# loicland/superpoint_graph

Measured on NVIDIA H100. Metric: spg_train_step_edges_plus_points_per_sec, higher is better.
Workload: dtype f32

## Files before the change

superpoint_graph_b200/csrc/tc_common.cuh:

```cuda
#pragma once
#include <cuda_runtime.h>
#include <stdint.h>

namespace spg {

__device__ __forceinline__ uint32_t smem_u32(const void* p) {
    return (uint32_t)__cvta_generic_to_shared(p);
}

__device__ __forceinline__ uint32_t to_tf32(float v) {
    return (__float_as_uint(v) + 0x1000u) & 0xffffe000u;
}

__device__ __forceinline__ void mbar_init(uint32_t bar, uint32_t count) {
    asm volatile("mbarrier.init.shared::cta.b64 [%0], %1;" ::"r"(bar), "r"(count));
}

__device__ __forceinline__ void mbar_wait(uint32_t bar, uint32_t parity) {
    asm volatile(
        "{\n\t"
        ".reg .pred P1;\n\t"
        "WAIT_LOOP:\n\t"
        "mbarrier.try_wait.parity.shared::cta.b64 P1, [%0], %1;\n\t"
        "@P1 bra WAIT_DONE;\n\t"
        "bra WAIT_LOOP;\n\t"
        "WAIT_DONE:\n\t"
        "}" ::"r"(bar), "r"(parity)
        : "memory");
}

__device__ __forceinline__ void mbar_arrive(uint32_t bar) {
    asm volatile("mbarrier.arrive.shared::cta.b64 _, [%0];" ::"r"(bar) : "memory");
}

__device__ __forceinline__ void mbar_expect_tx(uint32_t bar, uint32_t bytes) {
    asm volatile("mbarrier.arrive.expect_tx.shared::cta.b64 _, [%0], %1;" ::"r"(bar), "r"(bytes) : "memory");
}

__device__ __forceinline__ uint64_t wg_desc_k_sw128(uint32_t saddr) {
    return (uint64_t)((saddr >> 4) & 0x3FFFu) | ((uint64_t)1 << 16) | ((uint64_t)64 << 32) | ((uint64_t)1 << 62);
}

__device__ __forceinline__ uint32_t sw128_off(int row, int c16) {
    return (uint32_t)((row >> 3) * 1024 + (row & 7) * 128 + ((c16 ^ (row & 7)) << 4));
}

__device__ __forceinline__ void wg_fence() { asm volatile("wgmma.fence.sync.aligned;" ::: "memory"); }
__device__ __forceinline__ void wg_commit() { asm volatile("wgmma.commit_group.sync.aligned;" ::: "memory"); }
template <int N>
__device__ __forceinline__ void wg_wait() {
    asm volatile("wgmma.wait_group.sync.aligned %0;" ::"n"(N) : "memory");
}

template <int R>
__device__ __forceinline__ void wg_reg_fence(float (&d)[R]) {
#pragma unroll
    for (int i = 0; i < R; ++i) asm volatile("" : "+f"(d[i])::"memory");
}

template <int N>
__device__ __forceinline__ void wgmma_tf32(float (&d)[N / 2], uint64_t da, uint64_t db, uint32_t acc);
template <int N>
__device__ __forceinline__ void wgmma_bf16(float (&d)[N / 2], uint64_t da, uint64_t db, uint32_t acc);

template <>
__device__ __forceinline__ void wgmma_tf32<16>(float (&d)[8], uint64_t da, uint64_t db, uint32_t acc) {
    asm volatile(
        "{\n\t.reg .pred p;\n\tsetp.ne.b32 p, %10, 0;\n\t"
        "wgmma.mma_async.sync.aligned.m64n16k8.f32.tf32.tf32 {%0, %1, %2, %3, %4, %5, %6, %7}, %8, %9, p, 1, 1;\n\t}"
        : "+f"(d[0]), "+f"(d[1]), "+f"(d[2]), "+f"(d[3]), "+f"(d[4]), "+f"(d[5]), "+f"(d[6]), "+f"(d[7])
        : "l"(da), "l"(db), "r"(acc));
}

template <>
__device__ __forceinline__ void wgmma_tf32<32>(float (&d)[16], uint64_t da, uint64_t db, uint32_t acc) {
    asm volatile(
        "{\n\t.reg .pred p;\n\tsetp.ne.b32 p, %18, 0;\n\t"
        "wgmma.mma_async.sync.aligned.m64n32k8.f32.tf32.tf32 {%0, %1, %2, %3, %4, %5, %6, %7, %8, %9, %10, %11, %12, %13, %14, %15}, %16, %17, p, 1, 1;\n\t}"
        : "+f"(d[0]), "+f"(d[1]), "+f"(d[2]), "+f"(d[3]), "+f"(d[4]), "+f"(d[5]), "+f"(d[6]), "+f"(d[7]), "+f"(d[8]), "+f"(d[9]), "+f"(d[10]), "+f"(d[11]), "+f"(d[12]), "+f"(d[13]), "+f"(d[14]), "+f"(d[15])
        : "l"(da), "l"(db), "r"(acc));
}

template <>
__device__ __forceinline__ void wgmma_tf32<64>(float (&d)[32], uint64_t da, uint64_t db, uint32_t acc) {
    asm volatile(
        "{\n\t.reg .pred p;\n\tsetp.ne.b32 p, %34, 0;\n\t"
        "wgmma.mma_async.sync.aligned.m64n64k8.f32.tf32.tf32 {%0, %1, %2, %3, %4, %5, %6, %7, %8, %9, %10, %11, %12, %13, %14, %15, %16, %17, %18, %19, %20, %21, %22, %23, %24, %25, %26, %27, %28, %29, %30, %31}, %32, %33, p, 1, 1;\n\t}"
        : "+f"(d[0]), "+f"(d[1]), "+f"(d[2]), "+f"(d[3]), "+f"(d[4]), "+f"(d[5]), "+f"(d[6]), "+f"(d[7]), "+f"(d[8]), "+f"(d[9]), "+f"(d[10]), "+f"(d[11]), "+f"(d[12]), "+f"(d[13]), "+f"(d[14]), "+f"(d[15]), "+f"(d[16]), "+f"(d[17]), "+f"(d[18]), "+f"(d[19]), "+f"(d[20]), "+f"(d[21]), "+f"(d[22]), "+f"(d[23]), "+f"(d[24]), "+f"(d[25]), "+f"(d[26]), "+f"(d[27]), "+f"(d[28]), "+f"(d[29]), "+f"(d[30]), "+f"(d[31])
        : "l"(da), "l"(db), "r"(acc));
}

template <>
__device__ __forceinline__ void wgmma_tf32<128>(float (&d)[64], uint64_t da, uint64_t db, uint32_t acc) {
    asm volatile(
        "{\n\t.reg .pred p;\n\tsetp.ne.b32 p, %66, 0;\n\t"
        "wgmma.mma_async.sync.aligned.m64n128k8.f32.tf32.tf32 {%0, %1, %2, %3, %4, %5, %6, %7, %8, %9, %10, %11, %12, %13, %14, %15, %16, %17, %18, %19, %20, %21, %22, %23, %24, %25, %26, %27, %28, %29, %30, %31, %32, %33, %34, %35, %36, %37, %38, %39, %40, %41, %42, %43, %44, %45, %46, %47, %48, %49, %50, %51, %52, %53, %54, %55, %56, %57, %58, %59, %60, %61, %62, %63}, %64, %65, p, 1, 1;\n\t}"
        : "+f"(d[0]), "+f"(d[1]), "+f"(d[2]), "+f"(d[3]), "+f"(d[4]), "+f"(d[5]), "+f"(d[6]), "+f"(d[7]), "+f"(d[8]), "+f"(d[9]), "+f"(d[10]), "+f"(d[11]), "+f"(d[12]), "+f"(d[13]), "+f"(d[14]), "+f"(d[15]), "+f"(d[16]), "+f"(d[17]), "+f"(d[18]), "+f"(d[19]), "+f"(d[20]), "+f"(d[21]), "+f"(d[22]), "+f"(d[23]), "+f"(d[24]), "+f"(d[25]), "+f"(d[26]), "+f"(d[27]), "+f"(d[28]), "+f"(d[29]), "+f"(d[30]), "+f"(d[31]), "+f"(d[32]), "+f"(d[33]), "+f"(d[34]), "+f"(d[35]), "+f"(d[36]), "+f"(d[37]), "+f"(d[38]), "+f"(d[39]), "+f"(d[40]), "+f"(d[41]), "+f"(d[42]), "+f"(d[43]), "+f"(d[44]), "+f"(d[45]), "+f"(d[46]), "+f"(d[47]), "+f"(d[48]), "+f"(d[49]), "+f"(d[50]), "+f"(d[51]), "+f"(d[52]), "+f"(d[53]), "+f"(d[54]), "+f"(d[55]), "+f"(d[56]), "+f"(d[57]), "+f"(d[58]), "+f"(d[59]), "+f"(d[60]), "+f"(d[61]), "+f"(d[62]), "+f"(d[63])
        : "l"(da), "l"(db), "r"(acc));
}

template <>
__device__ __forceinline__ void wgmma_bf16<32>(float (&d)[16], uint64_t da, uint64_t db, uint32_t acc) {
    asm volatile(
        "{\n\t.reg .pred p;\n\tsetp.ne.b32 p, %18, 0;\n\t"
        "wgmma.mma_async.sync.aligned.m64n32k16.f32.bf16.bf16 {%0, %1, %2, %3, %4, %5, %6, %7, %8, %9, %10, %11, %12, %13, %14, %15}, %16, %17, p, 1, 1, 0, 0;\n\t}"
        : "+f"(d[0]), "+f"(d[1]), "+f"(d[2]), "+f"(d[3]), "+f"(d[4]), "+f"(d[5]), "+f"(d[6]), "+f"(d[7]), "+f"(d[8]), "+f"(d[9]), "+f"(d[10]), "+f"(d[11]), "+f"(d[12]), "+f"(d[13]), "+f"(d[14]), "+f"(d[15])
        : "l"(da), "l"(db), "r"(acc));
}

template <>
__device__ __forceinline__ void wgmma_bf16<64>(float (&d)[32], uint64_t da, uint64_t db, uint32_t acc) {
    asm volatile(
        "{\n\t.reg .pred p;\n\tsetp.ne.b32 p, %34, 0;\n\t"
        "wgmma.mma_async.sync.aligned.m64n64k16.f32.bf16.bf16 {%0, %1, %2, %3, %4, %5, %6, %7, %8, %9, %10, %11, %12, %13, %14, %15, %16, %17, %18, %19, %20, %21, %22, %23, %24, %25, %26, %27, %28, %29, %30, %31}, %32, %33, p, 1, 1, 0, 0;\n\t}"
        : "+f"(d[0]), "+f"(d[1]), "+f"(d[2]), "+f"(d[3]), "+f"(d[4]), "+f"(d[5]), "+f"(d[6]), "+f"(d[7]), "+f"(d[8]), "+f"(d[9]), "+f"(d[10]), "+f"(d[11]), "+f"(d[12]), "+f"(d[13]), "+f"(d[14]), "+f"(d[15]), "+f"(d[16]), "+f"(d[17]), "+f"(d[18]), "+f"(d[19]), "+f"(d[20]), "+f"(d[21]), "+f"(d[22]), "+f"(d[23]), "+f"(d[24]), "+f"(d[25]), "+f"(d[26]), "+f"(d[27]), "+f"(d[28]), "+f"(d[29]), "+f"(d[30]), "+f"(d[31])
        : "l"(da), "l"(db), "r"(acc));
}

template <>
__device__ __forceinline__ void wgmma_bf16<128>(float (&d)[64], uint64_t da, uint64_t db, uint32_t acc) {
    asm volatile(
        "{\n\t.reg .pred p;\n\tsetp.ne.b32 p, %66, 0;\n\t"
        "wgmma.mma_async.sync.aligned.m64n128k16.f32.bf16.bf16 {%0, %1, %2, %3, %4, %5, %6, %7, %8, %9, %10, %11, %12, %13, %14, %15, %16, %17, %18, %19, %20, %21, %22, %23, %24, %25, %26, %27, %28, %29, %30, %31, %32, %33, %34, %35, %36, %37, %38, %39, %40, %41, %42, %43, %44, %45, %46, %47, %48, %49, %50, %51, %52, %53, %54, %55, %56, %57, %58, %59, %60, %61, %62, %63}, %64, %65, p, 1, 1, 0, 0;\n\t}"
        : "+f"(d[0]), "+f"(d[1]), "+f"(d[2]), "+f"(d[3]), "+f"(d[4]), "+f"(d[5]), "+f"(d[6]), "+f"(d[7]), "+f"(d[8]), "+f"(d[9]), "+f"(d[10]), "+f"(d[11]), "+f"(d[12]), "+f"(d[13]), "+f"(d[14]), "+f"(d[15]), "+f"(d[16]), "+f"(d[17]), "+f"(d[18]), "+f"(d[19]), "+f"(d[20]), "+f"(d[21]), "+f"(d[22]), "+f"(d[23]), "+f"(d[24]), "+f"(d[25]), "+f"(d[26]), "+f"(d[27]), "+f"(d[28]), "+f"(d[29]), "+f"(d[30]), "+f"(d[31]), "+f"(d[32]), "+f"(d[33]), "+f"(d[34]), "+f"(d[35]), "+f"(d[36]), "+f"(d[37]), "+f"(d[38]), "+f"(d[39]), "+f"(d[40]), "+f"(d[41]), "+f"(d[42]), "+f"(d[43]), "+f"(d[44]), "+f"(d[45]), "+f"(d[46]), "+f"(d[47]), "+f"(d[48]), "+f"(d[49]), "+f"(d[50]), "+f"(d[51]), "+f"(d[52]), "+f"(d[53]), "+f"(d[54]), "+f"(d[55]), "+f"(d[56]), "+f"(d[57]), "+f"(d[58]), "+f"(d[59]), "+f"(d[60]), "+f"(d[61]), "+f"(d[62]), "+f"(d[63])
        : "l"(da), "l"(db), "r"(acc));
}


}
```

superpoint_graph_b200/csrc/tc_dw.cu:

```cuda
#include "common.cuh"
#include "tc_common.cuh"

namespace spg {

constexpr int DW_CONS_WARPS = 8, DW_PROD_WARPS = 4;
constexpr int DW_PROD_THREADS = DW_PROD_WARPS * 32;
constexpr int DW_THREADS = (DW_CONS_WARPS + DW_PROD_WARPS) * 32;
constexpr int DW_PTS = 32;
constexpr int DW_MAX_STAGES = 4;
constexpr int DW_SMEM_LIMIT = 232448;
constexpr int DW_STATIC_SMEM = 2048;

template <int CO, int CI>
struct DwCfg {
    static constexpr int A_BYTES = CO * DW_PTS * 4;
    static constexpr int B_BYTES = CI * DW_PTS * 4;
    static constexpr int STAGE_BYTES = 2 * A_BYTES + 2 * B_BYTES;
    static constexpr int FIT = (DW_SMEM_LIMIT - 1024 - DW_STATIC_SMEM) / STAGE_BYTES;
    static constexpr int STAGES = FIT < DW_MAX_STAGES ? FIT : DW_MAX_STAGES;
    static constexpr int SMEM = STAGES * STAGE_BYTES + 1024;
    static constexpr int A_F4 = CO * DW_PTS / 4 / DW_PROD_THREADS;
    static constexpr int B_F4 = CI * DW_PTS / 4 / DW_PROD_THREADS;
    static constexpr int PF_FIT = 24 / (A_F4 + B_F4);
    static constexpr int PF = PF_FIT < 1 ? 1 : (PF_FIT > 4 ? 4 : PF_FIT);
    static_assert(STAGES >= 2, "ring");
};

struct DwArgs {
    const float* dY;
    int64_t lddy;
    const float* P;
    int64_t ldp;
    const float *p_scale, *p_shift;
    int p_relu;
    float* partial;
    int64_t M;
    int64_t pts_per_cta;
};

template <int CO, int CI>
__global__ void __launch_bounds__(DW_THREADS, 1) tc_dw_kernel(const DwArgs p) {
    using Cfg = DwCfg<CO, CI>;
    constexpr int WM = CO >= 128 ? CO / 2 : 64;
    constexpr int WN = CO >= 128 ? CI : CI / 2;
    constexpr int MSUB = WM / 64;
    constexpr int A_BYTES = Cfg::A_BYTES, B_BYTES = Cfg::B_BYTES, STAGE_BYTES = Cfg::STAGE_BYTES;
    constexpr int STAGES = Cfg::STAGES, PF = Cfg::PF, A_F4 = Cfg::A_F4, B_F4 = Cfg::B_F4;
    static_assert(CO % 64 == 0 && CI % 32 == 0 && CI <= 128 && CO <= 256, "shape");

    extern __shared__ __align__(1024) uint8_t smem_raw[];
    uint8_t* smem = reinterpret_cast<uint8_t*>((reinterpret_cast<uintptr_t>(smem_raw) + 1023) & ~(uintptr_t)1023);
    __shared__ __align__(8) uint64_t bars[2 * DW_MAX_STAGES];
    __shared__ __align__(16) float sc_s[128], sh_s[128];
    static_assert(sizeof(bars) + sizeof(sc_s) + sizeof(sh_s) <= DW_STATIC_SMEM, "static shared memory");

    const int t = threadIdx.x;
    const int warp = t >> 5, lane = t & 31;
    const uint32_t bars_u32 = smem_u32(&bars[0]);
    auto bar_full = [&](int s) { return bars_u32 + 8u * (uint32_t)s; };
    auto bar_empty = [&](int s) { return bars_u32 + 8u * (uint32_t)(DW_MAX_STAGES + s); };
    if (t == 0) {
#pragma unroll
        for (int s = 0; s < STAGES; ++s) {
            mbar_init(bar_full(s), DW_PROD_WARPS);
            mbar_init(bar_empty(s), DW_CONS_WARPS);
        }
        asm volatile("fence.mbarrier_init.release.cluster;" ::: "memory");
    }
    SPG_PDL_ENTRY();

    const int64_t m_beg = (int64_t)blockIdx.x * p.pts_per_cta;
    const int64_t m_end = min(p.M, m_beg + p.pts_per_cta);
    const int nchunks = m_beg < m_end ? (int)((m_end - m_beg + DW_PTS - 1) / DW_PTS) : 0;

    const int ptid = t - DW_CONS_WARPS * 32;
    const int pt = (ptid >> 5) * 8 + (lane & 7), c40 = lane >> 3;
    float4 q[PF][A_F4 + B_F4];
    auto load_chunk = [&](int ch, float4 (&dst)[A_F4 + B_F4]) {
        const int64_t row = m_beg + (int64_t)ch * DW_PTS + pt;
        const bool ok = row < m_end;
        const float4* ga = reinterpret_cast<const float4*>(p.dY + row * p.lddy) + c40;
        const float4* gb = reinterpret_cast<const float4*>(p.P + row * p.ldp) + c40;
#pragma unroll
        for (int j = 0; j < A_F4; ++j) dst[j] = ok ? __ldg(ga + 4 * j) : make_float4(0.f, 0.f, 0.f, 0.f);
#pragma unroll
        for (int j = 0; j < B_F4; ++j) dst[A_F4 + j] = ok ? __ldg(gb + 4 * j) : make_float4(0.f, 0.f, 0.f, 0.f);
    };
    if (ptid >= 0) {
#pragma unroll
        for (int d = 0; d < PF; ++d) load_chunk(d, q[d]);
    }
    if (t < CI) {
        sc_s[t] = p.p_scale ? p.p_scale[t] : 1.f;
        sh_s[t] = p.p_shift ? p.p_shift[t] : 0.f;
    }
    __syncthreads();

    if (warp >= DW_CONS_WARPS) {
        const bool pro = p.p_scale || p.p_shift || p.p_relu;
        uint32_t soff[4];
#pragma unroll
        for (int e = 0; e < 4; ++e) soff[e] = sw128_off(4 * c40 + e, pt >> 2) + (uint32_t)(pt & 3) * 4u;
        auto st_shared = [](uint32_t addr, uint32_t v) {
            asm volatile("st.shared.b32 [%0], %1;" ::"r"(addr), "r"(v) : "memory");
        };
        auto split_store = [&](const uint32_t (&base)[4], uint32_t hi_off, uint32_t lo, int j, float4 v) {
            const float vv[4] = {v.x, v.y, v.z, v.w};
#pragma unroll
            for (int e = 0; e < 4; ++e) {
                const uint32_t addr = base[e] + hi_off + 2048u * (uint32_t)j;
                const uint32_t hi = to_tf32(vv[e]);
                st_shared(addr, hi);
                st_shared(addr + lo, to_tf32(vv[e] - __uint_as_float(hi)));
            }
        };
        const uint32_t smem_u = smem_u32(smem);
        int ch = 0, s = 0;
        uint32_t use = 0;
        auto produce = [&](float4 (&cur)[A_F4 + B_F4]) {
            if (use > 0) mbar_wait(bar_empty(s), (use - 1) & 1);
            uint32_t base[4];
#pragma unroll
            for (int e = 0; e < 4; ++e) base[e] = smem_u + (uint32_t)s * STAGE_BYTES + soff[e];
            const bool affine = pro && m_beg + (int64_t)ch * DW_PTS + pt < m_end;
#pragma unroll
            for (int j = 0; j < A_F4; ++j) split_store(base, 0u, A_BYTES, j, cur[j]);
#pragma unroll
            for (int j = 0; j < B_F4; ++j) {
                float4 v = cur[A_F4 + j];
                if (affine) {
                    const float4 sc = *reinterpret_cast<const float4*>(sc_s + (c40 + 4 * j) * 4);
                    const float4 sh = *reinterpret_cast<const float4*>(sh_s + (c40 + 4 * j) * 4);
                    v.x = fmaf(v.x, sc.x, sh.x);
                    v.y = fmaf(v.y, sc.y, sh.y);
                    v.z = fmaf(v.z, sc.z, sh.z);
                    v.w = fmaf(v.w, sc.w, sh.w);
                    if (p.p_relu) {
                        v.x = fmaxf(v.x, 0.f);
                        v.y = fmaxf(v.y, 0.f);
                        v.z = fmaxf(v.z, 0.f);
                        v.w = fmaxf(v.w, 0.f);
                    }
                }
                split_store(base, 2 * A_BYTES, B_BYTES, j, v);
            }
            load_chunk(ch + PF, cur);
            asm volatile("fence.proxy.async.shared::cta;" ::: "memory");
            __syncwarp();
            if (lane == 0) mbar_arrive(bar_full(s));
            ++ch;
            if (++s == STAGES) {
                s = 0;
                ++use;
            }
        };
        while (ch < nchunks) {
#pragma unroll
            for (int u = 0; u < PF; ++u) {
                produce(q[u]);
                if (ch >= nchunks) break;
            }
        }
    } else {
        const int g = warp >> 2, wl = warp & 3;
        float acc[MSUB][WN / 2];
#pragma unroll
        for (int m = 0; m < MSUB; ++m)
#pragma unroll
            for (int i = 0; i < WN / 2; ++i) acc[m][i] = 0.f;
        const int row_g = CO >= 128 ? g * WM : 0;
        const int col_g = CO >= 128 ? 0 : g * WN;
        const uint32_t smem_u = smem_u32(smem);

        int s = 0, s_prev = 0;
        uint32_t phase = 0;
        for (int ch = 0; ch < nchunks; ++ch) {
            mbar_wait(bar_full(s), phase);
            const uint32_t a_hi = smem_u + (uint32_t)s * STAGE_BYTES;
            const uint32_t ah = a_hi + (uint32_t)row_g * 128u, al = ah + A_BYTES;
            const uint32_t bh = a_hi + 2 * A_BYTES + (uint32_t)col_g * 128u, bl = bh + B_BYTES;
#pragma unroll
            for (int m = 0; m < MSUB; ++m) wg_reg_fence(acc[m]);
            wg_fence();
#pragma unroll
            for (int kb = 0; kb < DW_PTS / 8; ++kb) {
                const uint64_t dbh = wg_desc_k_sw128(bh + kb * 32), dbl = wg_desc_k_sw128(bl + kb * 32);
#pragma unroll
                for (int m = 0; m < MSUB; ++m) {
                    const uint64_t dah = wg_desc_k_sw128(ah + m * 64 * 128 + kb * 32);
                    const uint64_t dal = wg_desc_k_sw128(al + m * 64 * 128 + kb * 32);
                    wgmma_tf32<WN>(acc[m], dah, dbh, 1u);
                    wgmma_tf32<WN>(acc[m], dal, dbh, 1u);
                    wgmma_tf32<WN>(acc[m], dah, dbl, 1u);
                }
            }
            wg_commit();
            if (ch > 0) {
                wg_wait<1>();
                __syncwarp();
                if (lane == 0) mbar_arrive(bar_empty(s_prev));
            }
            s_prev = s;
            if (++s == STAGES) {
                s = 0;
                phase ^= 1u;
            }
        }
        wg_wait<0>();
#pragma unroll
        for (int m = 0; m < MSUB; ++m) wg_reg_fence(acc[m]);

        float* out = p.partial + (int64_t)blockIdx.x * CO * CI;
        const int r = lane >> 2, cq = 2 * (lane & 3);
#pragma unroll
        for (int m = 0; m < MSUB; ++m) {
            const int row = row_g + m * 64 + wl * 16 + r;
#pragma unroll
            for (int j = 0; j < WN / 8; ++j) {
                const int col = col_g + 8 * j + cq;
                *reinterpret_cast<float2*>(out + (int64_t)row * CI + col) =
                    make_float2(acc[m][4 * j], acc[m][4 * j + 1]);
                *reinterpret_cast<float2*>(out + (int64_t)(row + 8) * CI + col) =
                    make_float2(acc[m][4 * j + 2], acc[m][4 * j + 3]);
            }
        }
    }
}

template <int CO, int CI>
static int launch_dw(const DwArgs& a, int ctas, cudaStream_t s) {
    constexpr int smem = DwCfg<CO, CI>::SMEM;
    cudaError_t e = cudaFuncSetAttribute(tc_dw_kernel<CO, CI>, cudaFuncAttributeMaxDynamicSharedMemorySize, smem);
    if (e != cudaSuccess) return (int)e;
    SPG_LAUNCH(K_TC_DW, s, (tc_dw_kernel<CO, CI>), (unsigned)ctas, DW_THREADS, smem, a);
    return launch_status();
}

}

using namespace spg;

extern "C" {

int spg_tc_dw_supported(int64_t M, int co, int ci) {
    const bool co_ok = (co == 64 || co == 128 || co == 256);
    const bool ci_ok = (ci == 32 || ci == 64 || ci == 128);
    return (M >= DW_PTS && co_ok && ci_ok) ? 1 : 0;
}

int spg_tc_dw_ctas(int64_t M) {
    int64_t chunks = ceil_div64(M, DW_PTS);
    int64_t ctas = chunks < kNumSMs ? chunks : kNumSMs;
    return (int)(ctas < 1 ? 1 : ctas);
}

int spg_tc_dw(const float* dY, int64_t lddy, const float* P, int64_t ldp, const float* p_scale,
              const float* p_shift, int p_relu, float* dW, float* workspace, int64_t M, int co, int ci,
              spg_stream_t stream) {
    if (!dY || !P || !dW || !workspace || M <= 0) return SPG_E_BADARG;
    if (!spg_tc_dw_supported(M, co, ci)) return SPG_E_UNSUPPORTED;
    if ((lddy & 3) || (ldp & 3) || lddy < co || ldp < ci) return SPG_E_ALIGN;
    if (((uintptr_t)dY | (uintptr_t)P | (uintptr_t)workspace | (uintptr_t)p_scale | (uintptr_t)p_shift) & 15)
        return SPG_E_ALIGN;
    const int ctas = spg_tc_dw_ctas(M);
    DwArgs a;
    a.dY = dY; a.lddy = lddy; a.P = P; a.ldp = ldp; a.p_scale = p_scale; a.p_shift = p_shift;
    a.p_relu = p_relu; a.partial = workspace; a.M = M;
    cudaStream_t s = (cudaStream_t)stream;
    a.pts_per_cta = ceil_div64(ceil_div64(M, ctas), DW_PTS) * DW_PTS;
    int rc;
#define SPG_DW_CASE(CO_, CI_) \
    if (co == CO_ && ci == CI_) rc = launch_dw<CO_, CI_>(a, ctas, s); else
    SPG_DW_CASE(64, 32) SPG_DW_CASE(64, 64) SPG_DW_CASE(64, 128) SPG_DW_CASE(128, 32)
    SPG_DW_CASE(128, 64) SPG_DW_CASE(128, 128) SPG_DW_CASE(256, 32) SPG_DW_CASE(256, 64)
    SPG_DW_CASE(256, 128) rc = SPG_E_UNSUPPORTED;
#undef SPG_DW_CASE
    if (rc) return rc;
    return spg_splitk_reduce(workspace, ctas, co, ci, nullptr, dW, ci, stream);
}

}
```

Before: 47.68 million.

## Load dY operand directly into registers for wgmma A fragments in dW kernel

The weight-gradient kernel now has consumer warps load dY straight from global memory into register A-fragments, split them into tf32 hi/lo in registers, and feed register-sourced wgmma. This drops dY staging through shared memory, so stages hold only P and the ring is a fixed 4 stages. The output row mapping is permuted to match the fragment layout, and setmaxnreg rebalances registers between producer and consumer warps for large tiles. In exchange, consumers now sit on global-load latency and carry more register pressure, and the finer per-k-step wgmma commit/wait pattern adds synchronisation.

```diff
diff --git a/superpoint_graph_b200/csrc/tc_common.cuh b/superpoint_graph_b200/csrc/tc_common.cuh
--- a/superpoint_graph_b200/csrc/tc_common.cuh
+++ b/superpoint_graph_b200/csrc/tc_common.cuh
@@ -57,6 +57,11 @@
 #pragma unroll
     for (int i = 0; i < R; ++i) asm volatile("" : "+f"(d[i])::"memory");
 }
+template <int R>
+__device__ __forceinline__ void wg_reg_fence(uint32_t (&d)[R]) {
+#pragma unroll
+    for (int i = 0; i < R; ++i) asm volatile("" : "+r"(d[i])::"memory");
+}
 
 template <int N>
 __device__ __forceinline__ void wgmma_tf32(float (&d)[N / 2], uint64_t da, uint64_t db, uint32_t acc);
@@ -99,6 +104,45 @@
         : "l"(da), "l"(db), "r"(acc));
 }
 
+template <int N>
+__device__ __forceinline__ void wgmma_tf32(float (&d)[N / 2], const uint32_t (&a)[4], uint64_t db, uint32_t acc);
+
+template <>
+__device__ __forceinline__ void wgmma_tf32<16>(float (&d)[8], const uint32_t (&a)[4], uint64_t db, uint32_t acc) {
+    asm volatile(
+        "{\n\t.reg .pred p;\n\tsetp.ne.b32 p, %13, 0;\n\t"
+        "wgmma.mma_async.sync.aligned.m64n16k8.f32.tf32.tf32 {%0, %1, %2, %3, %4, %5, %6, %7}, {%8, %9, %10, %11}, %12, p, 1, 1;\n\t}"
+        : "+f"(d[0]), "+f"(d[1]), "+f"(d[2]), "+f"(d[3]), "+f"(d[4]), "+f"(d[5]), "+f"(d[6]), "+f"(d[7])
+        : "r"(a[0]), "r"(a[1]), "r"(a[2]), "r"(a[3]), "l"(db), "r"(acc));
+}
+
+template <>
+__device__ __forceinline__ void wgmma_tf32<32>(float (&d)[16], const uint32_t (&a)[4], uint64_t db, uint32_t acc) {
+    asm volatile(
+        "{\n\t.reg .pred p;\n\tsetp.ne.b32 p, %21, 0;\n\t"
+        "wgmma.mma_async.sync.aligned.m64n32k8.f32.tf32.tf32 {%0, %1, %2, %3, %4, %5, %6, %7, %8, %9, %10, %11, %12, %13, %14, %15}, {%16, %17, %18, %19}, %20, p, 1, 1;\n\t}"
+        : "+f"(d[0]), "+f"(d[1]), "+f"(d[2]), "+f"(d[3]), "+f"(d[4]), "+f"(d[5]), "+f"(d[6]), "+f"(d[7]), "+f"(d[8]), "+f"(d[9]), "+f"(d[10]), "+f"(d[11]), "+f"(d[12]), "+f"(d[13]), "+f"(d[14]), "+f"(d[15])
+        : "r"(a[0]), "r"(a[1]), "r"(a[2]), "r"(a[3]), "l"(db), "r"(acc));
+}
+
+template <>
+__device__ __forceinline__ void wgmma_tf32<64>(float (&d)[32], const uint32_t (&a)[4], uint64_t db, uint32_t acc) {
+    asm volatile(
+        "{\n\t.reg .pred p;\n\tsetp.ne.b32 p, %37, 0;\n\t"
+        "wgmma.mma_async.sync.aligned.m64n64k8.f32.tf32.tf32 {%0, %1, %2, %3, %4, %5, %6, %7, %8, %9, %10, %11, %12, %13, %14, %15, %16, %17, %18, %19, %20, %21, %22, %23, %24, %25, %26, %27, %28, %29, %30, %31}, {%32, %33, %34, %35}, %36, p, 1, 1;\n\t}"
+        : "+f"(d[0]), "+f"(d[1]), "+f"(d[2]), "+f"(d[3]), "+f"(d[4]), "+f"(d[5]), "+f"(d[6]), "+f"(d[7]), "+f"(d[8]), "+f"(d[9]), "+f"(d[10]), "+f"(d[11]), "+f"(d[12]), "+f"(d[13]), "+f"(d[14]), "+f"(d[15]), "+f"(d[16]), "+f"(d[17]), "+f"(d[18]), "+f"(d[19]), "+f"(d[20]), "+f"(d[21]), "+f"(d[22]), "+f"(d[23]), "+f"(d[24]), "+f"(d[25]), "+f"(d[26]), "+f"(d[27]), "+f"(d[28]), "+f"(d[29]), "+f"(d[30]), "+f"(d[31])
+        : "r"(a[0]), "r"(a[1]), "r"(a[2]), "r"(a[3]), "l"(db), "r"(acc));
+}
+
+template <>
+__device__ __forceinline__ void wgmma_tf32<128>(float (&d)[64], const uint32_t (&a)[4], uint64_t db, uint32_t acc) {
+    asm volatile(
+        "{\n\t.reg .pred p;\n\tsetp.ne.b32 p, %69, 0;\n\t"
+        "wgmma.mma_async.sync.aligned.m64n128k8.f32.tf32.tf32 {%0, %1, %2, %3, %4, %5, %6, %7, %8, %9, %10, %11, %12, %13, %14, %15, %16, %17, %18, %19, %20, %21, %22, %23, %24, %25, %26, %27, %28, %29, %30, %31, %32, %33, %34, %35, %36, %37, %38, %39, %40, %41, %42, %43, %44, %45, %46, %47, %48, %49, %50, %51, %52, %53, %54, %55, %56, %57, %58, %59, %60, %61, %62, %63}, {%64, %65, %66, %67}, %68, p, 1, 1;\n\t}"
+        : "+f"(d[0]), "+f"(d[1]), "+f"(d[2]), "+f"(d[3]), "+f"(d[4]), "+f"(d[5]), "+f"(d[6]), "+f"(d[7]), "+f"(d[8]), "+f"(d[9]), "+f"(d[10]), "+f"(d[11]), "+f"(d[12]), "+f"(d[13]), "+f"(d[14]), "+f"(d[15]), "+f"(d[16]), "+f"(d[17]), "+f"(d[18]), "+f"(d[19]), "+f"(d[20]), "+f"(d[21]), "+f"(d[22]), "+f"(d[23]), "+f"(d[24]), "+f"(d[25]), "+f"(d[26]), "+f"(d[27]), "+f"(d[28]), "+f"(d[29]), "+f"(d[30]), "+f"(d[31]), "+f"(d[32]), "+f"(d[33]), "+f"(d[34]), "+f"(d[35]), "+f"(d[36]), "+f"(d[37]), "+f"(d[38]), "+f"(d[39]), "+f"(d[40]), "+f"(d[41]), "+f"(d[42]), "+f"(d[43]), "+f"(d[44]), "+f"(d[45]), "+f"(d[46]), "+f"(d[47]), "+f"(d[48]), "+f"(d[49]), "+f"(d[50]), "+f"(d[51]), "+f"(d[52]), "+f"(d[53]), "+f"(d[54]), "+f"(d[55]), "+f"(d[56]), "+f"(d[57]), "+f"(d[58]), "+f"(d[59]), "+f"(d[60]), "+f"(d[61]), "+f"(d[62]), "+f"(d[63])
+        : "r"(a[0]), "r"(a[1]), "r"(a[2]), "r"(a[3]), "l"(db), "r"(acc));
+}
+
 template <>
 __device__ __forceinline__ void wgmma_bf16<32>(float (&d)[16], uint64_t da, uint64_t db, uint32_t acc) {
     asm volatile(
diff --git a/superpoint_graph_b200/csrc/tc_dw.cu b/superpoint_graph_b200/csrc/tc_dw.cu
--- a/superpoint_graph_b200/csrc/tc_dw.cu
+++ b/superpoint_graph_b200/csrc/tc_dw.cu
@@ -1,5 +1,7 @@
 #include "common.cuh"
 #include "tc_common.cuh"
+
+#include <type_traits>
 
 namespace spg {
 
@@ -7,23 +9,28 @@
 constexpr int DW_PROD_THREADS = DW_PROD_WARPS * 32;
 constexpr int DW_THREADS = (DW_CONS_WARPS + DW_PROD_WARPS) * 32;
 constexpr int DW_PTS = 32;
-constexpr int DW_MAX_STAGES = 4;
+constexpr int DW_KSTEPS = DW_PTS / 8;
+constexpr int DW_STAGES = 4;
 constexpr int DW_SMEM_LIMIT = 232448;
 constexpr int DW_STATIC_SMEM = 2048;
 
 template <int CO, int CI>
 struct DwCfg {
-    static constexpr int A_BYTES = CO * DW_PTS * 4;
+    static constexpr int WM = CO >= 128 ? CO / 2 : 64;
+    static constexpr int WN = CO >= 128 ? CI : CI / 2;
+    static constexpr int MSUB = WM / 64;
     static constexpr int B_BYTES = CI * DW_PTS * 4;
-    static constexpr int STAGE_BYTES = 2 * A_BYTES + 2 * B_BYTES;
-    static constexpr int FIT = (DW_SMEM_LIMIT - 1024 - DW_STATIC_SMEM) / STAGE_BYTES;
-    static constexpr int STAGES = FIT < DW_MAX_STAGES ? FIT : DW_MAX_STAGES;
-    static constexpr int SMEM = STAGES * STAGE_BYTES + 1024;
-    static constexpr int A_F4 = CO * DW_PTS / 4 / DW_PROD_THREADS;
+    static constexpr int STAGE_BYTES = 2 * B_BYTES;
+    static constexpr int SMEM = DW_STAGES * STAGE_BYTES + 1024;
+    static_assert(SMEM + DW_STATIC_SMEM <= DW_SMEM_LIMIT, "ring");
     static constexpr int B_F4 = CI * DW_PTS / 4 / DW_PROD_THREADS;
-    static constexpr int PF_FIT = 24 / (A_F4 + B_F4);
+    static constexpr bool REG_SPLIT = WM * WN > 128 * 64;
+    static constexpr int CONS_REGS = 224, PROD_REGS = 56;
+    static constexpr int PF_FIT = REG_SPLIT ? 1 : 24 / B_F4;
     static constexpr int PF = PF_FIT < 1 ? 1 : (PF_FIT > 4 ? 4 : PF_FIT);
-    static_assert(STAGES >= 2, "ring");
+    static constexpr int HL = WN * MSUB <= 64 ? 4 : 2;
+    static constexpr int RAW = MSUB == 1 ? 2 * DW_KSTEPS : 2;
+    static_assert(DW_KSTEPS % HL == 0 && (DW_KSTEPS % RAW == 0 || RAW == 2 * DW_KSTEPS), "A fragment rings");
 };
 
 struct DwArgs {
@@ -41,16 +48,14 @@
 template <int CO, int CI>
 __global__ void __launch_bounds__(DW_THREADS, 1) tc_dw_kernel(const DwArgs p) {
     using Cfg = DwCfg<CO, CI>;
-    constexpr int WM = CO >= 128 ? CO / 2 : 64;
-    constexpr int WN = CO >= 128 ? CI : CI / 2;
-    constexpr int MSUB = WM / 64;
-    constexpr int A_BYTES = Cfg::A_BYTES, B_BYTES = Cfg::B_BYTES, STAGE_BYTES = Cfg::STAGE_BYTES;
-    constexpr int STAGES = Cfg::STAGES, PF = Cfg::PF, A_F4 = Cfg::A_F4, B_F4 = Cfg::B_F4;
+    constexpr int WM = Cfg::WM, WN = Cfg::WN, MSUB = Cfg::MSUB;
+    constexpr int B_BYTES = Cfg::B_BYTES, STAGE_BYTES = Cfg::STAGE_BYTES;
+    constexpr int PF = Cfg::PF, B_F4 = Cfg::B_F4, HL = Cfg::HL, RAW = Cfg::RAW;
     static_assert(CO % 64 == 0 && CI % 32 == 0 && CI <= 128 && CO <= 256, "shape");
 
     extern __shared__ __align__(1024) uint8_t smem_raw[];
     uint8_t* smem = reinterpret_cast<uint8_t*>((reinterpret_cast<uintptr_t>(smem_raw) + 1023) & ~(uintptr_t)1023);
-    __shared__ __align__(8) uint64_t bars[2 * DW_MAX_STAGES];
+    __shared__ __align__(8) uint64_t bars[2 * DW_STAGES];
     __shared__ __align__(16) float sc_s[128], sh_s[128];
     static_assert(sizeof(bars) + sizeof(sc_s) + sizeof(sh_s) <= DW_STATIC_SMEM, "static shared memory");
 
@@ -58,10 +63,10 @@
     const int warp = t >> 5, lane = t & 31;
     const uint32_t bars_u32 = smem_u32(&bars[0]);
     auto bar_full = [&](int s) { return bars_u32 + 8u * (uint32_t)s; };
-    auto bar_empty = [&](int s) { return bars_u32 + 8u * (uint32_t)(DW_MAX_STAGES + s); };
+    auto bar_empty = [&](int s) { return bars_u32 + 8u * (uint32_t)(DW_STAGES + s); };
     if (t == 0) {
 #pragma unroll
-        for (int s = 0; s < STAGES; ++s) {
+        for (int s = 0; s < DW_STAGES; ++s) {
             mbar_init(bar_full(s), DW_PROD_WARPS);
             mbar_init(bar_empty(s), DW_CONS_WARPS);
         }
@@ -75,20 +80,40 @@
 
     const int ptid = t - DW_CONS_WARPS * 32;
     const int pt = (ptid >> 5) * 8 + (lane & 7), c40 = lane >> 3;
-    float4 q[PF][A_F4 + B_F4];
-    auto load_chunk = [&](int ch, float4 (&dst)[A_F4 + B_F4]) {
+    float4 q[PF][B_F4];
+    auto load_chunk = [&](int ch, float4 (&dst)[B_F4]) {
         const int64_t row = m_beg + (int64_t)ch * DW_PTS + pt;
         const bool ok = row < m_end;
-        const float4* ga = reinterpret_cast<const float4*>(p.dY + row * p.lddy) + c40;
         const float4* gb = reinterpret_cast<const float4*>(p.P + row * p.ldp) + c40;
 #pragma unroll
-        for (int j = 0; j < A_F4; ++j) dst[j] = ok ? __ldg(ga + 4 * j) : make_float4(0.f, 0.f, 0.f, 0.f);
-#pragma unroll
-        for (int j = 0; j < B_F4; ++j) dst[A_F4 + j] = ok ? __ldg(gb + 4 * j) : make_float4(0.f, 0.f, 0.f, 0.f);
+        for (int j = 0; j < B_F4; ++j) dst[j] = ok ? __ldg(gb + 4 * j) : make_float4(0.f, 0.f, 0.f, 0.f);
+    };
+    const int g = warp >> 2, wl = warp & 3;
+    const int a_co = (CO >= 128 ? g * WM : 0) + (wl * 8 + (lane >> 2)) * 2 * MSUB;
+    float a_raw[RAW][MSUB][4];
+    auto load_a = [&](int kstep, float (&dst)[MSUB][4]) {
+        const int64_t i0 = m_beg + (int64_t)kstep * 8 + (lane & 3);
+        const bool ok0 = i0 < m_end, ok1 = i0 + 4 < m_end;
+        const float* y0 = p.dY + i0 * p.lddy + a_co;
+        const float* y1 = y0 + 4 * p.lddy;
+        if constexpr (MSUB == 1) {
+            const float2 v0 = ok0 ? __ldg(reinterpret_cast<const float2*>(y0)) : make_float2(0.f, 0.f);
+            const float2 v1 = ok1 ? __ldg(reinterpret_cast<const float2*>(y1)) : make_float2(0.f, 0.f);
+            dst[0][0] = v0.x; dst[0][1] = v0.y; dst[0][2] = v1.x; dst[0][3] = v1.y;
+        } else {
+            static_assert(MSUB == 2, "A fragment loads");
+            const float4 v0 = ok0 ? __ldg(reinterpret_cast<const float4*>(y0)) : make_float4(0.f, 0.f, 0.f, 0.f);
+            const float4 v1 = ok1 ? __ldg(reinterpret_cast<const float4*>(y1)) : make_float4(0.f, 0.f, 0.f, 0.f);
+            dst[0][0] = v0.x; dst[0][1] = v0.y; dst[1][0] = v0.z; dst[1][1] = v0.w;
+            dst[0][2] = v1.x; dst[0][3] = v1.y; dst[1][2] = v1.z; dst[1][3] = v1.w;
+        }
     };
     if (ptid >= 0) {
 #pragma unroll
         for (int d = 0; d < PF; ++d) load_chunk(d, q[d]);
+    } else {
+#pragma unroll
+        for (int j = 0; j < RAW; ++j) load_a(j, a_raw[j]);
     }
     if (t < CI) {
         sc_s[t] = p.p_scale ? p.p_scale[t] : 1.f;
@@ -97,6 +122,7 @@
     __syncthreads();
 
     if (warp >= DW_CONS_WARPS) {
+        if constexpr (Cfg::REG_SPLIT) asm volatile("setmaxnreg.dec.sync.aligned.u32 %0;" ::"n"(Cfg::PROD_REGS));
         const bool pro = p.p_scale || p.p_shift || p.p_relu;
         uint32_t soff[4];
 #pragma unroll
@@ -104,30 +130,16 @@
         auto st_shared = [](uint32_t addr, uint32_t v) {
             asm volatile("st.shared.b32 [%0], %1;" ::"r"(addr), "r"(v) : "memory");
         };
-        auto split_store = [&](const uint32_t (&base)[4], uint32_t hi_off, uint32_t lo, int j, float4 v) {
-            const float vv[4] = {v.x, v.y, v.z, v.w};
-#pragma unroll
-            for (int e = 0; e < 4; ++e) {
-                const uint32_t addr = base[e] + hi_off + 2048u * (uint32_t)j;
-                const uint32_t hi = to_tf32(vv[e]);
-                st_shared(addr, hi);
-                st_shared(addr + lo, to_tf32(vv[e] - __uint_as_float(hi)));
-            }
-        };
         const uint32_t smem_u = smem_u32(smem);
         int ch = 0, s = 0;
         uint32_t use = 0;
-        auto produce = [&](float4 (&cur)[A_F4 + B_F4]) {
+        auto produce = [&](float4 (&cur)[B_F4]) {
             if (use > 0) mbar_wait(bar_empty(s), (use - 1) & 1);
-            uint32_t base[4];
-#pragma unroll
-            for (int e = 0; e < 4; ++e) base[e] = smem_u + (uint32_t)s * STAGE_BYTES + soff[e];
+            const uint32_t stage = smem_u + (uint32_t)s * STAGE_BYTES;
             const bool affine = pro && m_beg + (int64_t)ch * DW_PTS + pt < m_end;
 #pragma unroll
-            for (int j = 0; j < A_F4; ++j) split_store(base, 0u, A_BYTES, j, cur[j]);
-#pragma unroll
             for (int j = 0; j < B_F4; ++j) {
-                float4 v = cur[A_F4 + j];
+                float4 v = cur[j];
                 if (affine) {
                     const float4 sc = *reinterpret_cast<const float4*>(sc_s + (c40 + 4 * j) * 4);
                     const float4 sh = *reinterpret_cast<const float4*>(sh_s + (c40 + 4 * j) * 4);
@@ -142,14 +154,21 @@
                         v.w = fmaxf(v.w, 0.f);
                     }
                 }
-                split_store(base, 2 * A_BYTES, B_BYTES, j, v);
+                const float vv[4] = {v.x, v.y, v.z, v.w};
+#pragma unroll
+                for (int e = 0; e < 4; ++e) {
+                    const uint32_t addr = stage + soff[e] + 2048u * (uint32_t)j;
+                    const uint32_t hi = to_tf32(vv[e]);
+                    st_shared(addr, hi);
+                    st_shared(addr + B_BYTES, to_tf32(vv[e] - __uint_as_float(hi)));
+                }
             }
             load_chunk(ch + PF, cur);
             asm volatile("fence.proxy.async.shared::cta;" ::: "memory");
             __syncwarp();
             if (lane == 0) mbar_arrive(bar_full(s));
             ++ch;
-            if (++s == STAGES) {
+            if (++s == DW_STAGES) {
                 s = 0;
                 ++use;
             }
@@ -162,65 +181,93 @@
             }
         }
     } else {
-        const int g = warp >> 2, wl = warp & 3;
+        if constexpr (Cfg::REG_SPLIT) asm volatile("setmaxnreg.inc.sync.aligned.u32 %0;" ::"n"(Cfg::CONS_REGS));
         float acc[MSUB][WN / 2];
 #pragma unroll
         for (int m = 0; m < MSUB; ++m)
 #pragma unroll
             for (int i = 0; i < WN / 2; ++i) acc[m][i] = 0.f;
-        const int row_g = CO >= 128 ? g * WM : 0;
+        uint32_t a_hi[HL][MSUB][4], a_lo[HL][MSUB][4];
+#pragma unroll
+        for (int m = 0; m < MSUB; ++m) wg_reg_fence(acc[m]);
         const int col_g = CO >= 128 ? 0 : g * WN;
         const uint32_t smem_u = smem_u32(smem);
 
         int s = 0, s_prev = 0;
         uint32_t phase = 0;
-        for (int ch = 0; ch < nchunks; ++ch) {
+        auto consume = [&](int ch, auto par) {
+            constexpr int PAR = decltype(par)::value;
             mbar_wait(bar_full(s), phase);
-            const uint32_t a_hi = smem_u + (uint32_t)s * STAGE_BYTES;
-            const uint32_t ah = a_hi + (uint32_t)row_g * 128u, al = ah + A_BYTES;
-            const uint32_t bh = a_hi + 2 * A_BYTES + (uint32_t)col_g * 128u, bl = bh + B_BYTES;
-#pragma unroll
-            for (int m = 0; m < MSUB; ++m) wg_reg_fence(acc[m]);
-            wg_fence();
-#pragma unroll
-            for (int kb = 0; kb < DW_PTS / 8; ++kb) {
+            const uint32_t bh = smem_u + (uint32_t)s * STAGE_BYTES + (uint32_t)col_g * 128u, bl = bh + B_BYTES;
+#pragma unroll
+            for (int kb = 0; kb < DW_KSTEPS; ++kb) {
+                const int h = kb % HL, r = (PAR * DW_KSTEPS + kb) % RAW;
+                wg_wait<HL - 1>();
+#pragma unroll
+                for (int m = 0; m < MSUB; ++m) {
+                    wg_reg_fence(a_hi[h][m]);
+                    wg_reg_fence(a_lo[h][m]);
+                }
+                if (kb == HL - 1 && ch > 0) {
+                    __syncwarp();
+                    if (lane == 0) mbar_arrive(bar_empty(s_prev));
+                }
+#pragma unroll
+                for (int m = 0; m < MSUB; ++m)
+#pragma unroll
+                    for (int e = 0; e < 4; ++e) {
+                        const float v = a_raw[r][m][e];
+                        const uint32_t hi = to_tf32(v);
+                        a_hi[h][m][e] = hi;
+                        a_lo[h][m][e] = to_tf32(v - __uint_as_float(hi));
+                    }
+                load_a(ch * DW_KSTEPS + kb + RAW, a_raw[r]);
+                wg_fence();
                 const uint64_t dbh = wg_desc_k_sw128(bh + kb * 32), dbl = wg_desc_k_sw128(bl + kb * 32);
 #pragma unroll
                 for (int m = 0; m < MSUB; ++m) {
-                    const uint64_t dah = wg_desc_k_sw128(ah + m * 64 * 128 + kb * 32);
-                    const uint64_t dal = wg_desc_k_sw128(al + m * 64 * 128 + kb * 32);
-                    wgmma_tf32<WN>(acc[m], dah, dbh, 1u);
-                    wgmma_tf32<WN>(acc[m], dal, dbh, 1u);
-                    wgmma_tf32<WN>(acc[m], dah, dbl, 1u);
-                }
-            }
-            wg_commit();
-            if (ch > 0) {
-                wg_wait<1>();
-                __syncwarp();
-                if (lane == 0) mbar_arrive(bar_empty(s_prev));
+                    wgmma_tf32<WN>(acc[m], a_hi[h][m], dbh, 1u);
+                    wgmma_tf32<WN>(acc[m], a_lo[h][m], dbh, 1u);
+                    wgmma_tf32<WN>(acc[m], a_hi[h][m], dbl, 1u);
+                }
+                wg_commit();
             }
             s_prev = s;
-            if (++s == STAGES) {
+            if (++s == DW_STAGES) {
                 s = 0;
                 phase ^= 1u;
             }
+        };
+        if constexpr (RAW > DW_KSTEPS) {
+            for (int ch = 0; ch < nchunks; ch += 2) {
+                consume(ch, std::integral_constant<int, 0>());
+                if (ch + 1 < nchunks) consume(ch + 1, std::integral_constant<int, 1>());
+            }
+        } else {
+            for (int ch = 0; ch < nchunks; ++ch) consume(ch, std::integral_constant<int, 0>());
         }
         wg_wait<0>();
 #pragma unroll
         for (int m = 0; m < MSUB; ++m) wg_reg_fence(acc[m]);
+#pragma unroll
+        for (int h = 0; h < HL; ++h)
+#pragma unroll
+            for (int m = 0; m < MSUB; ++m) {
+                wg_reg_fence(a_hi[h][m]);
+                wg_reg_fence(a_lo[h][m]);
+            }
 
         float* out = p.partial + (int64_t)blockIdx.x * CO * CI;
-        const int r = lane >> 2, cq = 2 * (lane & 3);
+        const int cq = 2 * (lane & 3);
 #pragma unroll
         for (int m = 0; m < MSUB; ++m) {
-            const int row = row_g + m * 64 + wl * 16 + r;
+            const int row = a_co + 2 * m;
 #pragma unroll
             for (int j = 0; j < WN / 8; ++j) {
                 const int col = col_g + 8 * j + cq;
                 *reinterpret_cast<float2*>(out + (int64_t)row * CI + col) =
                     make_float2(acc[m][4 * j], acc[m][4 * j + 1]);
-                *reinterpret_cast<float2*>(out + (int64_t)(row + 8) * CI + col) =
+                *reinterpret_cast<float2*>(out + (int64_t)(row + 1) * CI + col) =
                     make_float2(acc[m][4 * j + 2], acc[m][4 * j + 3]);
             }
         }
```

Measured after the change: 50.22 million (median of 6 runs). 5.3% higher.
